# VatsalSy/gerris-fft-particles

Hardware: AMD Instinct MI355X
Metric: Mcell-steps/s (projection+advection), 3D 256^3 uniform (higher is better)
Workload: dtype f64; 1 GPU; 3-D periodic Taylor-Green, 256^3 per GPU, default projection/advection parameters (SURVEY 8d config C); relax_mode=exact, parallelism=1 box, rccl_world_size=0

## Files before the change

### gerris-fft-particles_amd/csrc/gfship_internal.hpp

```cpp
#pragma once

#include <hip/hip_runtime.h>
#include <cstdio>
#include <cstdarg>
#include <cstring>
#include <vector>
#include <deque>
#include <string>
#include <type_traits>
#include "gfship.h"
#include "switches.hpp"
#include "cell_update.hpp"

namespace gfship {

struct Layout {
  int n = 0;
  int px = 0;
  int xo = 1;
  int rows = 0;
  int dim = 3;
  long sy = 0;
  long sz = 0;
  size_t total = 0;
// ... 76 lines not shown
  double * h_pinned = nullptr;
  gfship_exchange_fn exchange = nullptr; void * exchange_ctx = nullptr;
  gfship_reduce_fn reduce = nullptr;     void * reduce_ctx = nullptr;
  bool has_external = false;
  void * comm = nullptr;
  int overlap = 0;
  int lat_rank = -1, lat_n = 0, lat_b[3] = { 1, 1, 1 };
  gfship_gather_fn gather = nullptr; void * gather_ctx = nullptr;
  double * lat_res = nullptr, * lat_xch = nullptr;
  unsigned * lat_bar = nullptr;
  size_t lat_res_doubles = 0, lat_xch_doubles = 0;
  double * gfv_send[6] = {}, * gfv_recv[6] = {};
  double src[3] = { 0., 0., 0. };
  unsigned long long n_lattice_cycles = 0, n_fused_mpi = 0;
  unsigned long long kc[GFSHIP_KC_COUNT] = {};
  bool lattice_attr_set = false;
  void * mpi_plan[GFSHIP_MAXLEVEL + 1] = {};
  gfship_field dp_cache = -1;
  int skew_resident = -1;
  int patch_resident = 0;
  bool no_fused_godunov = false;
  bool no_fused_loop = false;
  bool force_hyperplane = false;
  bool unit_weights = false;
  bool weighted = false;
  unsigned long weights_stamp = 0;
  gfship_field wf[6] = {-1, -1, -1, -1, -1, -1};
  gfship::SkewPlan skew[GFSHIP_MAXLEVEL + 1];
  double diff_w[GFSHIP_MAXLEVEL + 1] = {};
  double * cfl_partial = nullptr;
  size_t cfl_nblocks = 0, cfl_used = 0;
  bool cfl_dirty = false;
  bool coarse_attr_set = false;
  gfship_field res_cache = -1;
  bool diff_ready = false;
  int diff_kind = 1;
  int patch_call = -1;
};

namespace gfship {

void set_error (const char * fmt, ...);
int  hip_fail (hipError_t e, const char * what, const char * file, int line);

inline int before_write (gfship_domain * dom)
{
  return dom->before_write ? dom->before_write (dom->before_write_ctx) : GFSHIP_OK;
}

#define GFSHIP_HIP(call) do { hipError_t e_ = (call); \
    if (e_ != hipSuccess) return gfship::hip_fail (e_, #call, __FILE__, __LINE__); } while (0)

inline hipError_t stream_wait_spin (hipStream_t st)
{
  hipError_t e;
  while ((e = hipStreamQuery (st)) == hipErrorNotReady)
    ;
  return e;
}

template <class F> inline void with_bools (F && f) { f (); }
template <class F, class... B> inline void with_bools (F && f, bool b0, B... rest)
{
  if (b0) with_bools ([&] (auto... r) { f (std::true_type {}, r...); }, rest...);
  else    with_bools ([&] (auto... r) { f (std::false_type {}, r...); }, rest...);
}

template <class F, class... B> inline void with_kind (F && f, int kind, B... bools)
{
  auto k = [&] (auto K) { with_bools ([&] (auto... r) { f (K, r...); }, bools...); };
  if (kind == 3)      k (std::integral_constant<int, 3> {});
  else if (kind == 2) k (std::integral_constant<int, 2> {});
  else if (kind)      k (std::integral_constant<int, 1> {});
  else                k (std::integral_constant<int, 0> {});
}

#define GFSHIP_CHECK(cond, code, ...) do { if (!(cond)) { \
    gfship::set_error (__VA_ARGS__); return (code); } } while (0)

Field * get_field (gfship_domain * dom, gfship_field f);
int coarse_flush (gfship_domain * dom, Field * F, int level, bool leaf_write = false);
inline long ncells (const Layout & L) {
  return L.dim == 3 ? (long) L.n*L.n*L.n : (long) L.n*L.n;
}

int launch_bc (gfship_domain * dom, Field * v, Field * v1, int level, int homogeneous);
bool all_sides_periodic (const gfship_domain * dom);

__device__ __forceinline__ void periodic_images (const Layout & L, double * __restrict__ a, int i, int j, int k,
						  double v)
{
  const int n = L.n;
  if (i == 1) a[L.idx (n + 1, j, k)] = v;
  if (i == n) a[L.idx (0, j, k)] = v;
  if (j == 1) a[L.idx (i, n + 1, k)] = v;
  if (j == n) a[L.idx (i, 0, k)] = v;
  if (k == 1) a[L.idx (i, j, n + 1)] = v;
  if (k == n) a[L.idx (i, j, 0)] = v;
}
int call_exchange (gfship_domain * dom, double * ptr, int level, int kind);
int bc_mpi_begin (gfship_domain * dom, Field * v1, int level);
int bc_mpi_end (gfship_domain * dom, Field * v, Field * v1, int level, int homogeneous);
int call_reduce (gfship_domain * dom, double * vals, int n, int op);
int call_reduce_norm (gfship_domain * dom, double * sums, int nsum, double * mx);
int comm_exchange (gfship_domain * dom, double * a, int level, int kind);
int comm_exchange_raw (gfship_domain * dom, double * const send[6], double * const recv[6], size_t count);
int comm_migrate (gfship_domain * dom, int rs, const int nsend[6], const double * const send[6],
		  int nrecv[6], std::vector<double> recv[6]);
int comm_allgather (gfship_domain * dom, const double * send, double * recv, size_t count);
int multi_buffers (gfship_domain * dom);
int launch_bc_multi (gfship_domain * dom, Field * const * v, int nf, int level, int homogeneous);
int call_gather (gfship_domain * dom, const double * send, double * recv, size_t count);
int comm_exchange_begin (gfship_domain * dom, double * a, int level);
int comm_exchange_end (gfship_domain * dom, double * a, int level);
int comm_reduce (gfship_domain * dom, double * sums, int nsum, double * maxs, int nmax,
		 double * mins, int nmin);
void comm_free (gfship_domain * dom);
int launch_relax_exact (gfship_domain * dom, unsigned dimension, int level, double omega,
			double * u, const double * rhs, const double * dia,
			const RelaxOp * op = nullptr);
int launch_relax_mpi_first (gfship_domain * dom, unsigned dimension, int level, double omega,
			    double * u, const double * rhs, const double * dia, const RelaxOp * op,
			    int (* after_shell) (void *), void * ctx);
void mpi_order_free (gfship_domain * dom);
int launch_relax_loop_small (gfship_domain * dom, unsigned dimension, int level, double omega,
			     Field * dp, Field * ubc, const double * rhs, const double * dia,
			     unsigned nrelax, bool * done, const RelaxOp * op = nullptr);
int coarse_cycle_top (gfship_domain * dom, int minlevel);
int lattice_cycle_top (gfship_domain * dom, int minlevel, Field * dia);
int lattice_check_error (gfship_domain * dom);
int launch_lattice_cycle (gfship_domain * dom, unsigned dimension, double omega, int lmin, int ltop,
			  const unsigned * nrelax, Field * dp, Field * ubc, Field * res);
int launch_coarse_cycle (gfship_domain * dom, unsigned dimension, double omega, int lmin, int ltop,
			 const unsigned * nrelax, Field * dp, Field * ubc, Field * res, Field * dia);
int launch_relax_redblack (gfship_domain * dom, unsigned dimension, int level, double omega,
			   double * u, const double * rhs, const double * dia);
int launch_residual (gfship_domain * dom, int level, const double * u, const double * rhs,
		     const double * dia, double * res);
int launch_residual_weighted (gfship_domain * dom, int level, const double * u, const double * rhs,
			      const double * dia, double * res);
int launch_poisson_weights (gfship_domain * dom, double * const alpha[3]);
int launch_diffusion_weights (gfship_domain * dom, double * const D[3], double cdt);
int alloc_weights (gfship_domain * dom);
RelaxOp weighted_op (gfship_domain * dom, int level);
int launch_restrict (gfship_domain * dom, unsigned dimension, int level_coarse, double * v_coarse,
		     const double * v_fine);
int launch_prolongate (gfship_domain * dom, int level_coarse, const double * v_coarse,
		       double * v_fine);
int launch_correct (gfship_domain * dom, int level, double * u, const double * dp);
int launch_fill (gfship_domain * dom, int level, double * a, double value);
int launch_residual_norm (gfship_domain * dom, int level, const double * u, const double * rhs,
			  const double * dia, double * res, double scale, double weight,
			  double * out , bool dia_zero = false);
int launch_norm_async (gfship_domain * dom, int level, const double * a, double scale, double weight);
int launch_norm (gfship_domain * dom, int level, const double * a, double scale, double weight,
		 double out[5] );

int launch_face_interp_un (gfship_domain * dom, double * const u[3], double * const un[3]);
int launch_divergence (gfship_domain * dom, double * const un[3], double * div, double dt);
int launch_correct_un (gfship_domain * dom, const double * p, double * const un[3], double dt);
int launch_centered_gradient (gfship_domain * dom, const double * p, double * const g[3]);
int launch_correct_centered (gfship_domain * dom, double * const u[3], double * const g[3], double dt);
int launch_correct_centered_coarse (gfship_domain * dom, double * const u[3], double * const g[3],
				    double dt, double * const uc[3]);
int launch_coarse_init_from (gfship_domain * dom, Field * const * v, int nf, int top);
int launch_coarse_init_levels (gfship_domain * dom, Field * const * v, int nf, int top, int bottom);
// ... 84 lines not shown
```

### gerris-fft-particles_amd/csrc/poisson_kernels.hip

```cpp
#include "gfship_internal.hpp"
#include "cell_loop.hpp"
#include "relax_skew.hpp"
#include <algorithm>
#include <cstdlib>

namespace gfship {

template <int DIM, int OP>
__device__ __forceinline__ double relax_value (const double * __restrict__ u, long c, long sy, long sz,
					       double rhs, double dia, unsigned dimension,
					       double omega, double w, double h2, const W6 * wf = nullptr)
{
  return cell_update<DIM, OP> (kind_weights<OP> (w, ArrayW { wf, c }), ArrayU { u, c, sy, sz }, rhs, dia, u + c,
			       dimension, omega, h2);
}

__device__ __forceinline__ double relax_value_six (const double * __restrict__ u, long c, long sy, long sz,
						    double rhs)
{
  return cell_update_six (ArrayU { u, c, sy, sz }, rhs);
}

template <int DIM, int OP>
__global__ void __launch_bounds__(256)
// ... 1400 lines not shown
    for (int q = 0; q < 4; q++) {
      r0 += sh[0][q]; r1 += sh[1][q]; r2 += sh[2][q]; r3 = fmax (r3, sh[3][q]); r4 += sh[4][q];
    }
    out[0] = r0; out[1] = r1; out[2] = r2; out[3] = r3; out[4] = r4;
  }
}

static bool power_of_two (double x)
{
  int e;
  return x > 0. && frexp (x, &e) == 0.5;
}
#define NORM_PARTIAL_LAUNCH() do {					\
    if (power_of_two (scale))						\
      hipLaunchKernelGGL (norm_partial_kernel<true>, dim3 (nblocks), dim3 (block), 0, dom->stream, \
			  L, a, scale, weight, partial);		\
    else								\
      hipLaunchKernelGGL (norm_partial_kernel<false>, dim3 (nblocks), dim3 (block), 0, dom->stream, \
			  L, a, scale, weight, partial);		\
  } while (0)

int launch_norm_async (gfship_domain * dom, int level, const double * a, double scale, double weight)
{
  const Layout & L = dom->lay[level];
  long nrows = L.dim == 3 ? (long) L.n*L.n : L.n;
  int block = L.n >= 256 ? 256 : L.n >= 128 ? 128 : 64;
  int nblocks = (int) (nrows > 1024 ? 1024 : nrows);
  double * partial = dom->d_scratch;
  double * result = dom->h_pinned + 8;
  NORM_PARTIAL_LAUNCH ();
  hipLaunchKernelGGL (norm_final_kernel, dim3 (1), dim3 (256), 0, dom->stream,
		      partial, nblocks, result);
  GFSHIP_HIP (hipGetLastError ());
  return GFSHIP_OK;
}

int launch_norm (gfship_domain * dom, int level, const double * a, double scale, double weight,
		 double out[5])
{
  const Layout & L = dom->lay[level];
  long nrows = L.dim == 3 ? (long) L.n*L.n : L.n;
  int block = L.n >= 256 ? 256 : L.n >= 128 ? 128 : 64;
  int nblocks = (int) (nrows > 1024 ? 1024 : nrows);
  double * partial = dom->d_scratch;
  double * result = dom->h_pinned;
  NORM_PARTIAL_LAUNCH ();
  hipLaunchKernelGGL (norm_final_kernel, dim3 (1), dim3 (256), 0, dom->stream,
		      partial, nblocks, result);
  GFSHIP_HIP (hipGetLastError ());
  GFSHIP_HIP (stream_wait_spin (dom->stream));
  memcpy (out, dom->h_pinned, 5*sizeof (double));
  return GFSHIP_OK;
}

template <int DIM>
__global__ void __launch_bounds__(256)
residual_norm_kernel (Layout L, const double * __restrict__ u, const double * __restrict__ rhs,
		      const double * __restrict__ dia, double * __restrict__ res, double inv,
		      double weight, double * __restrict__ partial)
{
  const int n = L.n;
  const long nrows = DIM == 3 ? (long) n*n : n;
  double s0 = 0., s1 = 0., s2 = 0., s3 = 0., s4 = 0.;
  for (long r = blockIdx.x; r < nrows; r += gridDim.x) {
    const int j = (int) (r % n) + 1, k = DIM == 3 ? (int) (r / n) + 1 : 0;
    const long row = L.idx (1, j, k);
    for (int i = threadIdx.x; i < n; i += blockDim.x) {
      const long c = row + i;
      const FaceSums f = face_sums<DIM> (UnitW {}, ArrayU { u, c, L.sy, L.sz }, dia ? dia[c] : 0.);
      const double raw = residual_close (f.a, f.b, rhs[c], u[c]);
      res[c] = raw;
      double val = raw*inv;
      s0 += weight*val;
      val = fabs (val);
      s3 = fmax (s3, val);
      s1 += weight*val;
      s2 += weight*val*val;
      s4 += raw;
    }
  }
  block_norm_sums (s0, s1, s2, s3, s4, partial, blockIdx.x);
}

template <bool NORM>
__global__ void __launch_bounds__(256)
residual_norm2_kernel (Layout L, const double * __restrict__ u, const double * __restrict__ rhs,
		       const double * __restrict__ dia, double * __restrict__ res, double inv,
		       double weight, double * __restrict__ partial)
{
  typedef double d2 __attribute__((ext_vector_type(2)));
  const int n = L.n, half = n >> 1;
  const long nitems = (long) n*n*half;
  double s0 = 0., s1 = 0., s2 = 0., s3 = 0., s4 = 0.;
  for (long it = (long) blockIdx.x*blockDim.x + threadIdx.x; it < nitems; it += (long) gridDim.x*blockDim.x) {
    const int pr = (int) (it % half);
    const long r = it / half;
    const int j = (int) (r % n) + 1, k = (int) (r / n) + 1;
    const long c = L.idx (1 + 2*pr, j, k);
    const d2 uc = *(const d2 *) (u + c);
    const double ul = u[c - 1], ur = u[c + 2];
    const d2 ut = *(const d2 *) (u + c + L.sy), ub = *(const d2 *) (u + c - L.sy);
    const d2 uf = *(const d2 *) (u + c + L.sz), uk = *(const d2 *) (u + c - L.sz);
    const d2 rh = *(const d2 *) (rhs + c);
    d2 di = { 0., 0. };
    if (dia) di = *(const d2 *) (dia + c);
    d2 out;
    {
      double a = di.x, b = 0.;
      a += 1.; b += 1.*uc.y;
      a += 1.; b += 1.*ul;
      a += 1.; b += 1.*ut.x;
      a += 1.; b += 1.*ub.x;
      a += 1.; b += 1.*uf.x;
      a += 1.; b += 1.*uk.x;
      out.x = rh.x - (b - uc.x*a);
    }
    {
      double a = di.y, b = 0.;
      a += 1.; b += 1.*ur;
      a += 1.; b += 1.*uc.x;
      a += 1.; b += 1.*ut.y;
      a += 1.; b += 1.*ub.y;
      a += 1.; b += 1.*uf.y;
      a += 1.; b += 1.*uk.y;
      out.y = rh.y - (b - uc.y*a);
    }
    *(d2 *) (res + c) = out;
    if (NORM)
#pragma unroll
    for (int e = 0; e < 2; e++) {
      const double raw = e ? out.y : out.x;
      double val = raw*inv;
      s0 += weight*val;
      val = fabs (val);
      s3 = fmax (s3, val);
      s1 += weight*val;
      s2 += weight*val*val;
      s4 += raw;
    }
  }
  if (!NORM) return;
  __shared__ double sh[5][4];
  s0 = wave_sum (s0); s1 = wave_sum (s1); s2 = wave_sum (s2); s3 = wave_max (s3); s4 = wave_sum (s4);
  int w = threadIdx.x >> 6, lane = threadIdx.x & 63;
  if (lane == 0) { sh[0][w] = s0; sh[1][w] = s1; sh[2][w] = s2; sh[3][w] = s3; sh[4][w] = s4; }
  __syncthreads ();
  if (threadIdx.x == 0) {
    int nw = blockDim.x >> 6;
    double r0 = 0., r1 = 0., r2 = 0., r3 = 0., r4 = 0.;
    for (int q = 0; q < nw; q++) {
      r0 += sh[0][q]; r1 += sh[1][q]; r2 += sh[2][q]; r3 = fmax (r3, sh[3][q]); r4 += sh[4][q];
    }
    double * p = partial + 5*(size_t) blockIdx.x;
    p[0] = r0; p[1] = r1; p[2] = r2; p[3] = r3; p[4] = r4;
  }
}

int launch_residual_norm (gfship_domain * dom, int level, const double * u, const double * rhs,
			  const double * dia, double * res, double scale, double weight,
			  double * out, bool dia_zero)
{
  const Layout & L = dom->lay[level];
  if (!power_of_two (scale)) {
    int r = launch_residual (dom, level, u, rhs, dia, res);
    if (r) return r;
    return out ? launch_norm (dom, level, res, scale, weight, out) :
      launch_norm_async (dom, level, res, scale, weight);
  }
  long nrows = L.dim == 3 ? (long) L.n*L.n : L.n;
  int block = L.n >= 256 ? 256 : L.n >= 128 ? 128 : 64;
  int rn_blocks = dom->sw.rn_blocks;
  if (rn_blocks < 64 || rn_blocks > 8192) rn_blocks = 4096;
  int nblocks = (int) (nrows > rn_blocks ? rn_blocks : nrows);
  double * partial = dom->d_scratch;
  double * result = out ? dom->h_pinned : dom->h_pinned + 8;
  const bool rn_pairs = dom->sw.residual_pairs;
  if (dom->dim == 3 && L.n >= 64) dom->kc[rn_pairs ? GFSHIP_KC_RESIDUAL_PAIRS : GFSHIP_KC_RESIDUAL_SCALAR]++;
  if (dom->dim == 3 && L.n >= 64 && rn_pairs) {
    const long nitems = (long) L.n*L.n*(L.n/2);
    long nb = (nitems + 255)/256;
    nblocks = (int) (nb > rn_blocks ? rn_blocks : nb);
    hipLaunchKernelGGL (residual_norm2_kernel<true>, dim3 (nblocks), dim3 (256), 0, dom->stream, L, u,
			rhs, dia_zero ? nullptr : dia, res, 1./scale, weight, partial);
  }
  else
    with_bools ([&] (auto D3) {
      hipLaunchKernelGGL (residual_norm_kernel<decltype (D3)::value ? 3 : 2>, dim3 (nblocks), dim3 (block), 0,
			  dom->stream, L, u, rhs, dia_zero ? nullptr : dia, res, 1./scale, weight, partial);
    }, dom->dim == 3);
  hipLaunchKernelGGL (norm_final_kernel, dim3 (1), dim3 (256), 0, dom->stream,
		      partial, nblocks, result);
  GFSHIP_HIP (hipGetLastError ());
  dom->kc[GFSHIP_KC_RN_BLOCKS_LIMIT] = rn_blocks;
  if ((unsigned long long) nblocks > dom->kc[GFSHIP_KC_RN_BLOCKS_MAX])
    dom->kc[GFSHIP_KC_RN_BLOCKS_MAX] = nblocks;
  if (out) {
    GFSHIP_HIP (stream_wait_spin (dom->stream));
    memcpy (out, dom->h_pinned, 5*sizeof (double));
  }
  return GFSHIP_OK;
}

struct MpiOrderPlan {
  int * cells = nullptr;
  std::vector<int> first;
  int shell_steps = 0;
};

template <int DIM, int OP>
__global__ void __launch_bounds__(256)
relax_listed_kernel (const int * __restrict__ cells, int count, long sy, long sz,
		     unsigned dimension, double omega, double w, double h2,
		     double * __restrict__ u, const double * __restrict__ rhs,
		     const double * __restrict__ dia)
{
  const int q = blockIdx.x*blockDim.x + threadIdx.x;
  if (q >= count) return;
  const long c = cells[q];
  u[c] = relax_value<DIM, OP> (u, c, sy, sz, rhs[c], dia[c], dimension, omega, w, h2);
}

static inline unsigned long long morton_key (int dim, int level, int I, int J, int K)
{
  unsigned long long m = 0;
  for (int b = level - 1; b >= 0; b--) {
    unsigned n = ((I >> b) & 1) | (((J >> b) & 1) << 1) | (dim == 3 ? ((K >> b) & 1) << 2 : 0);
    m = (m << (dim == 3 ? 3 : 2)) | n;
  }
  return m;
}

void mpi_order_free (gfship_domain * dom)
{
  for (int l = 0; l <= GFSHIP_MAXLEVEL; l++)
    if (dom->mpi_plan[l]) {
      MpiOrderPlan * P = (MpiOrderPlan *) dom->mpi_plan[l];
// ... 121 lines not shown
```

### gerris-fft-particles_amd/csrc/timestep_kernels.hip

```cpp
#include "gfship_internal.hpp"
#include "cell_loop.hpp"
#include <cfloat>

namespace gfship {

#define EXT_PROLOGUE(L)							\
  int i = blockIdx.x*blockDim.x + threadIdx.x;				\
  int j = blockIdx.y;							\
  int k = (L).dim == 3 ? blockIdx.z : 0;				\
  if (i > (L).n) return;						\
  long c = (L).idx (i, j, k)

static inline void ext_grid (const Layout & L, dim3 * grid, dim3 * block)
{
  int b = L.n >= 256 ? 256 : L.n >= 128 ? 128 : 64;
  *block = dim3 (b);
  *grid = dim3 ((L.n + 1 + b - 1)/b, L.n + 1, L.dim == 3 ? L.n + 1 : 1);
}

struct Ptr3  { double * p[3]; };
struct CPtr3 { const double * p[3]; };
struct Ptr6  { double * p[6]; };
struct CPtr6 { const double * p[6]; };
struct Visc3 { double d[3]; double g[3]; };
// ... 107 lines not shown
	const long c = L.idx (2*i - 1, 2*j - dy, 2*k - dz);
	const d2 a = *(const d2 *) (u.p[cc] + c), b = *(const d2 *) (g.p[cc] + c);
	d2 r;
	r.x = a.x - b.x*dt; r.y = a.y - b.y*dt;
	*(d2 *) (u.p[cc] + c) = r;
	x[dz][dy][0] = r.x; x[dz][dy][1] = r.y;
      }
    double val = 0., sa = 0.;
#pragma unroll
    for (int id = 0; id < 8; id++) {
      val += x[(id >> 2) & 1][(id >> 1) & 1][id & 1]*1.;
      sa += 1.;
    }
    uc.p[cc][Lc.idx (i, j, k)] = val/sa;
  }
}

template <int DIM, bool FUSE_U>
__global__ void __launch_bounds__(256)
project_correct_kernel (Layout L, const double * __restrict__ p, Ptr3 un, Ptr3 g, Ptr3 u,
			double dt, double * __restrict__ partial_max)
{
  const int i1 = blockIdx.x*blockDim.x + threadIdx.x + 1;
  const int j = blockIdx.y;
  const int k = DIM == 3 ? blockIdx.z : 0;
  const int n = L.n;
  const double rn = (double) n;
  const long off[3] = { 1, L.sy, L.sz };
  double mx = 0.;
  auto body = [&] (int i) {
    const long c = L.idx (i, j, k);
    const bool interior = i >= 1 && j >= 1 && (DIM == 2 || k >= 1);
#pragma unroll
    for (int cc = 0; cc < DIM; cc++) {
      const bool valid = face_valid<DIM> (n, cc, i, j, k);
      if (valid || interior) {
	double dpp = (1.*p[c + off[cc]] - 1.*p[c])*rn;
	dpp /= 1.;
	if (valid) {
	  double w = un.p[cc][c];
	  w -= dpp*dt;
	  un.p[cc][c] = w;
	  mx = fmax (mx, fabs (w));
	}
	if (interior) {
	  double dpm = (1.*p[c] - 1.*p[c - off[cc]])*rn;
	  dpm /= 1.;
	  double v = 0.;
	  v += dpm*1.;
	  v += dpp*1.;
	  double gg = v/2.;
	  g.p[cc][c] = gg;
	  if (FUSE_U) {
	    double w = u.p[cc][c];
	    w -= gg*dt;
	    u.p[cc][c] = w;
	    mx = fmax (mx, fabs (1.*w));
	  }
	}
      }
    }
  };
  if (i1 <= n) {
    body (i1);
    if (i1 == 1)
      body (0);
  }
  if (partial_max) {
    __shared__ double sh[4];
    mx = wave_max (mx);
    if ((threadIdx.x & 63) == 0) sh[threadIdx.x >> 6] = mx;
    __syncthreads ();
    if (threadIdx.x == 0) {
      double r = sh[0];
      for (int q = 1; q < (int) (blockDim.x >> 6); q++) r = fmax (r, sh[q]);
      if (r > 0.)
	atomicMax ((unsigned long long *) partial_max +
		   ((blockIdx.x + gridDim.x*(blockIdx.y + (size_t) gridDim.y*blockIdx.z)) & 1023),
		   (unsigned long long) __double_as_longlong (r));
    }
  }
}

__global__ void __launch_bounds__(128)
face_interp_div2_kernel (Layout L, CPtr3 u, double * __restrict__ div, double dt)
{
  typedef double d2 __attribute__((ext_vector_type(2)));
  const int i1 = 2*(blockIdx.x*blockDim.x + threadIdx.x) + 1;
  const int j = blockIdx.y + 1, k = blockIdx.z + 1;
  if (i1 > L.n) return;
  const double h = 1./L.n;
  const long c = L.idx (i1, j, k);
  const long off[3] = { 1, L.sy, L.sz };
  d2 D = { 0., 0. };
#pragma unroll
  for (int cc = 0; cc < 3; cc++) {
    const d2 U = *(const d2 *) (u.p[cc] + c);
    d2 Un, Um;
    if (cc == 0) { Un.x = U.y; Un.y = u.p[0][c + 2]; Um.x = u.p[0][c - 1]; Um.y = U.x; }
    else { Un = *(const d2 *) (u.p[cc] + c + off[cc]); Um = *(const d2 *) (u.p[cc] + c - off[cc]); }
    {
      const double unp = face_interp (U.x, Un.x), unm = face_interp (Um.x, U.x);
      D.x += 1.*unp*1.;
      D.x += -1.*unm*1.;
    }
    {
      const double unp = face_interp (U.y, Un.y), unm = face_interp (Um.y, U.y);
      D.y += 1.*unp*1.;
      D.y += -1.*unm*1.;
    }
  }
  d2 out;
  { const double v = D.x*h; out.x = v/dt; }
  { const double v = D.y*h; out.y = v/dt; }
  *(d2 *) (div + c) = out;
}

__device__ __forceinline__ void periodic_images_pair (const Layout & L, double * __restrict__ a, long c,
						       int i1, int j, int k, double vx, double vy)
{
  typedef double d2 __attribute__((ext_vector_type(2)));
  const int n = L.n;
  const d2 V = { vx, vy };
  if (i1 == 1) a[c + n] = vx;
  if (i1 + 1 == n) a[c + 1 - n] = vy;
  if (j == 1) *(d2 *) (a + c + n*L.sy) = V;
  if (j == n) *(d2 *) (a + c - n*L.sy) = V;
  if (k == 1) *(d2 *) (a + c + n*L.sz) = V;
  if (k == n) *(d2 *) (a + c - n*L.sz) = V;
}

template <bool PER>
__global__ void __launch_bounds__(128)
project_correct2_kernel (Layout L, const double * __restrict__ p, Ptr3 un, Ptr3 g, double dt)
{
  typedef double d2 __attribute__((ext_vector_type(2)));
  const int i1 = 2*(blockIdx.x*blockDim.x + threadIdx.x) + 1;
  const int j = blockIdx.y, k = blockIdx.z;
  const int n = L.n;
  const double rn = (double) n;
  const long off[3] = { 1, L.sy, L.sz };
  auto body = [&] (int i) {
    const long c = L.idx (i, j, k);
    const bool interior = i >= 1 && j >= 1 && k >= 1;
#pragma unroll
    for (int cc = 0; cc < 3; cc++) {
      const bool valid = face_valid<3> (n, cc, i, j, k);
      if (valid || interior) {
	double dpp = (1.*p[c + off[cc]] - 1.*p[c])*rn;
	dpp /= 1.;
	if (valid) {
	  double w = un.p[cc][c];
	  w -= dpp*dt;
	  un.p[cc][c] = w;
	}
	if (interior) {
	  double dpm = (1.*p[c] - 1.*p[c - off[cc]])*rn;
	  dpm /= 1.;
	  double v = 0.;
	  v += dpm*1.;
	  v += dpp*1.;
	  g.p[cc][c] = v/2.;
	}
      }
    }
  };
  if (i1 > n) return;
  if (j >= 1 && k >= 1) {
    const long c = L.idx (i1, j, k);
    const d2 P = *(const d2 *) (p + c);
    const double pl = p[c - 1], pr = p[c + 2];
    const d2 Pn[3] = { { P.y, pr }, *(const d2 *) (p + c + L.sy), *(const d2 *) (p + c + L.sz) };
    const d2 Pm[3] = { { pl, P.x }, *(const d2 *) (p + c - L.sy), *(const d2 *) (p + c - L.sz) };
#pragma unroll
    for (int cc = 0; cc < 3; cc++) {
      d2 W = *(const d2 *) (un.p[cc] + c), G;
#pragma unroll
      for (int e = 0; e < 2; e++) {
	const double pc = e ? P.y : P.x, pn = e ? Pn[cc].y : Pn[cc].x, pm = e ? Pm[cc].y : Pm[cc].x;
	double dpp = (1.*pn - 1.*pc)*rn;
	dpp /= 1.;
	double w = e ? W.y : W.x;
	w -= dpp*dt;
	double dpm = (1.*pc - 1.*pm)*rn;
	dpm /= 1.;
	double v = 0.;
	v += dpm*1.;
	v += dpp*1.;
	if (e) { W.y = w; G.y = v/2.; } else { W.x = w; G.x = v/2.; }
      }
      *(d2 *) (un.p[cc] + c) = W;
      *(d2 *) (g.p[cc] + c) = G;
      if (PER) periodic_images_pair (L, g.p[cc], c, i1, j, k, G.x, G.y);
    }
  }
  else {
    body (i1);
    if (i1 + 1 <= n) body (i1 + 1);
  }
  if (i1 == 1)
    body (0);
}

template <bool PER>
__global__ void __launch_bounds__(128)
project_correct_lazy2_kernel (Layout L, const double * __restrict__ p, CPtr3 u, Ptr3 g, Ptr3 uo,
			      double dt, double * __restrict__ partial_max)
{
  typedef double d2 __attribute__((ext_vector_type(2)));
  const int i1 = 2*(blockIdx.x*blockDim.x + threadIdx.x) + 1;
  const int j = blockIdx.y, k = blockIdx.z;
  const int n = L.n;
  const double rn = (double) n;
  const long off[3] = { 1, L.sy, L.sz };
  double mx = 0.;
  auto body = [&] (int i) {
    const long c = L.idx (i, j, k);
    const bool interior = i >= 1 && j >= 1 && k >= 1;
#pragma unroll
    for (int cc = 0; cc < 3; cc++) {
      const bool valid = face_valid<3> (n, cc, i, j, k);
      if (valid || interior) {
	double dpp = (1.*p[c + off[cc]] - 1.*p[c])*rn;
	dpp /= 1.;
	const double uc = u.p[cc][c];
	if (valid) {
	  double w = face_interp (uc, u.p[cc][c + off[cc]]);
	  w -= dpp*dt;
	  mx = fmax (mx, fabs (w));
	}
	if (interior) {
	  double dpm = (1.*p[c] - 1.*p[c - off[cc]])*rn;
	  dpm /= 1.;
	  double v = 0.;
	  v += dpm*1.;
	  v += dpp*1.;
	  double gg = v/2.;
	  g.p[cc][c] = gg;
	  double w = uc;
	  w -= gg*dt;
	  uo.p[cc][c] = w;
	  mx = fmax (mx, fabs (1.*w));
	}
      }
    }
  };
  if (i1 <= n) {
    if (j >= 1 && k >= 1) {
      const long c = L.idx (i1, j, k);
      const d2 P = *(const d2 *) (p + c);
      const double pl = p[c - 1], pr = p[c + 2];
      const d2 Pn[3] = { { P.y, pr }, *(const d2 *) (p + c + L.sy), *(const d2 *) (p + c + L.sz) };
      const d2 Pm[3] = { { pl, P.x }, *(const d2 *) (p + c - L.sy), *(const d2 *) (p + c - L.sz) };
#pragma unroll
      for (int cc = 0; cc < 3; cc++) {
	const d2 U = *(const d2 *) (u.p[cc] + c);
	d2 Un;
	if (cc == 0) { Un.x = U.y; Un.y = u.p[0][c + 2]; }
	else Un = *(const d2 *) (u.p[cc] + c + off[cc]);
	d2 G, W;
#pragma unroll
	for (int e = 0; e < 2; e++) {
	  const double pc = e ? P.y : P.x, pn = e ? Pn[cc].y : Pn[cc].x, pm = e ? Pm[cc].y : Pm[cc].x;
	  const double uc = e ? U.y : U.x, un_ = e ? Un.y : Un.x;
	  double dpp = (1.*pn - 1.*pc)*rn;
	  dpp /= 1.;
	  double w = face_interp (uc, un_);
	  w -= dpp*dt;
	  mx = fmax (mx, fabs (w));
	  double dpm = (1.*pc - 1.*pm)*rn;
	  dpm /= 1.;
	  double v = 0.;
	  v += dpm*1.;
	  v += dpp*1.;
	  const double gg = v/2.;
	  double w2 = uc;
	  w2 -= gg*dt;
	  mx = fmax (mx, fabs (1.*w2));
	  if (e) { G.y = gg; W.y = w2; } else { G.x = gg; W.x = w2; }
	}
	*(d2 *) (g.p[cc] + c) = G;
	*(d2 *) (uo.p[cc] + c) = W;
	if (PER) {
	  periodic_images_pair (L, g.p[cc], c, i1, j, k, G.x, G.y);
	  periodic_images_pair (L, uo.p[cc], c, i1, j, k, W.x, W.y);
	}
      }
    }
    else {
      body (i1);
      if (i1 + 1 <= n) body (i1 + 1);
    }
    if (i1 == 1)
      body (0);
  }
  if (partial_max) {
    __shared__ double sh[4];
    mx = wave_max (mx);
    if ((threadIdx.x & 63) == 0) sh[threadIdx.x >> 6] = mx;
    __syncthreads ();
    if (threadIdx.x == 0) {
      double r = sh[0];
      for (int q = 1; q < (int) (blockDim.x >> 6); q++) r = fmax (r, sh[q]);
      if (r > 0.)
	atomicMax ((unsigned long long *) partial_max +
		   ((blockIdx.x + gridDim.x*(blockIdx.y + (size_t) gridDim.y*blockIdx.z)) & 1023),
		   (unsigned long long) __double_as_longlong (r));
    }
  }
}

struct W6t { const double * p[6]; };

template <int DIM>
__global__ void __launch_bounds__(256)
project_correct_weighted_kernel (Layout L, const double * __restrict__ p, Ptr3 un, Ptr3 g, Ptr3 u,
				 double dt, W6t wf)
{
  const int i1 = blockIdx.x*blockDim.x + threadIdx.x + 1;
  const int j = blockIdx.y;
  const int k = DIM == 3 ? blockIdx.z : 0;
  const int n = L.n;
  const double rn = (double) n;
  const long off[3] = { 1, L.sy, L.sz };
  auto body = [&] (int i) {
    const long c = L.idx (i, j, k);
    const int q[3] = { i, j, k };
    const bool interior = i >= 1 && j >= 1 && (DIM == 2 || k >= 1);
#pragma unroll
    for (int cc = 0; cc < DIM; cc++) {
      const bool valid = face_valid<DIM> (n, cc, i, j, k);
      if (valid || interior) {
	const double wp = q[cc] >= 1 ? wf.p[2*cc][c] : wf.p[2*cc + 1][c + off[cc]];
	double dpp = (wp*p[c + off[cc]] - wp*p[c])*rn;
	dpp /= 1.;
	if (valid && un.p[cc]) {
	  double w = un.p[cc][c];
	  w -= dpp*dt;
	  un.p[cc][c] = w;
	}
	if (interior) {
	  const double wm = q[cc] >= 2 ? wf.p[2*cc][c - off[cc]] : wf.p[2*cc + 1][c];
	  double dpm = (wm*p[c] - wm*p[c - off[cc]])*rn;
	  dpm /= 1.;
	  double v = 0.;
	  v += dpm*1.;
	  v += dpp*1.;
	  double gg = v/2.;
	  g.p[cc][c] = gg;
	  if (u.p[cc]) {
	    double w = u.p[cc][c];
	    w -= gg*dt;
	    u.p[cc][c] = w;
	  }
	}
      }
    }
  };
  if (i1 <= n) {
    body (i1);
    if (i1 == 1)
      body (0);
  }
}

template <int DIM>
__global__ void __launch_bounds__(256)
project_correct_lazy_kernel (Layout L, const double * __restrict__ p, CPtr3 u, Ptr3 g, Ptr3 uo,
			     double dt, double * __restrict__ partial_max)
{
  const int i1 = blockIdx.x*blockDim.x + threadIdx.x + 1;
  const int j = blockIdx.y;
  const int k = DIM == 3 ? blockIdx.z : 0;
  const int n = L.n;
  const double rn = (double) n;
  const long off[3] = { 1, L.sy, L.sz };
  double mx = 0.;
  auto body = [&] (int i) {
    const long c = L.idx (i, j, k);
    const bool interior = i >= 1 && j >= 1 && (DIM == 2 || k >= 1);
#pragma unroll
    for (int cc = 0; cc < DIM; cc++) {
      const bool valid = face_valid<DIM> (n, cc, i, j, k);
      if (valid || interior) {
	double dpp = (1.*p[c + off[cc]] - 1.*p[c])*rn;
	dpp /= 1.;
	const double uc = u.p[cc][c];
	if (valid) {
	  double w = face_interp (uc, u.p[cc][c + off[cc]]);
// ... 2262 lines not shown
  dim3 grid ((nface + block - 1)/block, 2*dom->dim);
  DISPATCH (dom, face_bc_kernel, grid, dim3 (block), L, bc, (const double *) v->lev[dom->depth],
	    m6 (fv), cmask);
  if (dom->has_external)
    for (int e = 0; e < 2*dom->dim; e++)
      if (dom->side[e ^ 1] == GFSHIP_SIDE_EXTERNAL && (cmask & (1 << (e/2)))) {
	int r = call_exchange (dom, fv[e], dom->depth, 1 + e);
	if (r) return r;
      }
  return GFSHIP_OK;
}

int launch_predict_un (gfship_domain * dom, int cc, const double * uc, double * const fv[6],
		       double * unc)
{
  const Layout & L = dom->lay[dom->depth];
  dim3 grid, block;
  ext_grid (L, &grid, &block);
  DISPATCH (dom, predict_un_kernel, grid, block, L, cc, uc, (const double *) fv[2*cc],
	    (const double *) fv[2*cc + 1], unc);
  return GFSHIP_OK;
}

int launch_flux_update (gfship_domain * dom, bool velocity, double * v, double * const un[3],
			double * const fv[6], const double * gm, const double * gc, double dt, double gsrc)
{
  const Layout & L = dom->lay[dom->depth];
  dim3 grid, block;
  cell_grid (L, &grid, &block);
  if (dom->dim == 3) {
    if (velocity)
      hipLaunchKernelGGL ((flux_update_kernel<3, true>), grid, block, 0, dom->stream,
			  L, v, c3 (un), c6 (fv), gm, gc, dt, gsrc);
    else
      hipLaunchKernelGGL ((flux_update_kernel<3, false>), grid, block, 0, dom->stream,
			  L, v, c3 (un), c6 (fv), gm, gc, dt, gsrc);
  }
  else {
    if (velocity)
      hipLaunchKernelGGL ((flux_update_kernel<2, true>), grid, block, 0, dom->stream,
			  L, v, c3 (un), c6 (fv), gm, gc, dt, gsrc);
    else
      hipLaunchKernelGGL ((flux_update_kernel<2, false>), grid, block, 0, dom->stream,
			  L, v, c3 (un), c6 (fv), gm, gc, dt, gsrc);
  }
  GFSHIP_HIP (hipGetLastError ());
  return GFSHIP_OK;
}

static inline void ext1_grid (const Layout & L, dim3 * grid, dim3 * block)
{
  int b = L.n >= 256 ? 256 : L.n >= 128 ? 128 : 64;
  *block = dim3 (b);
  *grid = dim3 ((L.n + b - 1)/b, L.n + 1, L.dim == 3 ? L.n + 1 : 1);
}

int launch_project_correct (gfship_domain * dom, const double * p, double * const un[3],
			    double * const g[3], double * const u[3] , double dt,
			    bool want_max, bool * ghosts_done)
{
  if (ghosts_done) *ghosts_done = false;
  const Layout & L = dom->lay[dom->depth];
  dim3 grid, block;
  ext1_grid (L, &grid, &block);
  double * pm = nullptr;
  if (want_max) {
    const size_t nb = 1024;
    if (!dom->cfl_partial) {
      GFSHIP_HIP (hipMalloc ((void **) &dom->cfl_partial, nb*sizeof (double)));
      GFSHIP_HIP (hipMemsetAsync (dom->cfl_partial, 0, nb*sizeof (double), dom->stream));
      dom->cfl_nblocks = nb;
    }
    dom->cfl_used = nb;
    if (dom->cfl_dirty)
      GFSHIP_HIP (hipMemsetAsync (dom->cfl_partial, 0, nb*sizeof (double), dom->stream));
    dom->cfl_dirty = true;
    pm = dom->cfl_partial;
  }
  Ptr3 none = { { nullptr, nullptr, nullptr } };
  const bool pairs = dom->sw.project_pairs;
  const bool pairs_apply = dom->dim == 3 && !u && !pm && L.n >= 64 && L.n % 2 == 0;
  if (pairs_apply) dom->kc[pairs ? GFSHIP_KC_PROJECT_PAIRS : GFSHIP_KC_PROJECT_SCALAR]++;
  if (pairs_apply && pairs) {
    const int b = 128, half = L.n/2;
    const bool per = ghosts_done && all_sides_periodic (dom);
    with_bools ([&] (auto PER) {
      hipLaunchKernelGGL (project_correct2_kernel<decltype (PER)::value>, dim3 ((half + b - 1)/b, L.n + 1, L.n + 1), dim3 (b), 0,
			  dom->stream, L, p, m3 (un), m3 (g), dt);
    }, per);
    GFSHIP_HIP (hipGetLastError ());
    if (per) *ghosts_done = true;
    return GFSHIP_OK;
  }
  with_bools ([&] (auto D3, auto U) {
    hipLaunchKernelGGL ((project_correct_kernel<decltype (D3)::value ? 3 : 2, decltype (U)::value>), grid, block, 0, dom->stream,
			L, p, m3 (un), m3 (g), u ? m3 (u) : none, dt, pm);
  }, dom->dim == 3, u != nullptr);
  GFSHIP_HIP (hipGetLastError ());
  return GFSHIP_OK;
}

int launch_project_correct_weighted (gfship_domain * dom, const double * p, double * const un[3] ,
				     double * const g[3], double * const u[3] , double dt)
{
  const int Lv = dom->depth;
  const Layout & L = dom->lay[Lv];
  dim3 grid, block;
  ext1_grid (L, &grid, &block);
  W6t wf;
  for (int d = 0; d < 6; d++)
    wf.p[d] = d < 2*dom->dim ? dom->fields[dom->wf[d]].lev[Lv] : nullptr;
  Ptr3 none = { { nullptr, nullptr, nullptr } };
  if (dom->dim == 3)
    hipLaunchKernelGGL ((project_correct_weighted_kernel<3>), grid, block, 0, dom->stream, L, p,
			un ? m3 (un) : none, m3 (g), u ? m3 (u) : none, dt, wf);
  else
    hipLaunchKernelGGL ((project_correct_weighted_kernel<2>), grid, block, 0, dom->stream, L, p,
			un ? m3 (un) : none, m3 (g), u ? m3 (u) : none, dt, wf);
  GFSHIP_HIP (hipGetLastError ());
  return GFSHIP_OK;
}

int launch_cfl_from_max (gfship_domain * dom, double * cfl2)
{
  const Layout & L = dom->lay[dom->depth];
  double * result = dom->h_pinned;
  hipLaunchKernelGGL (cfl_from_max_kernel, dim3 (1), dim3 (256), 0, dom->stream, dom->cfl_partial,
		      (int) dom->cfl_used, 1./L.n, result);
  dom->cfl_dirty = false;
  GFSHIP_HIP (hipGetLastError ());
  GFSHIP_HIP (stream_wait_spin (dom->stream));
  *cfl2 = dom->h_pinned[0];
  return call_reduce (dom, cfl2, 1, 2);
}

int launch_face_interp_div (gfship_domain * dom, double * const u[3], double * const un[3],
			    double * div, double dt)
{
  const Layout & L = dom->lay[dom->depth];
  dim3 grid, block;
  ext1_grid (L, &grid, &block);
  Ptr3 none = { { nullptr, nullptr, nullptr } };
  const bool pairs = dom->sw.project_pairs;
  const bool pairs_apply = !un && dom->dim == 3 && L.n >= 64 && L.n % 2 == 0;
  if (pairs_apply) dom->kc[pairs ? GFSHIP_KC_PROJECT_PAIRS : GFSHIP_KC_PROJECT_SCALAR]++;
  if (pairs_apply && pairs) {
    const int b = 128, half = L.n/2;
    hipLaunchKernelGGL (face_interp_div2_kernel, dim3 ((half + b - 1)/b, L.n, L.n), dim3 (b), 0, dom->stream, L, c3 (u), div, dt);
  }
  else
    with_bools ([&] (auto D3, auto UN) {
      hipLaunchKernelGGL ((face_interp_div_kernel<decltype (D3)::value ? 3 : 2, decltype (UN)::value>), grid, block, 0, dom->stream,
			  L, c3 (u), un ? m3 (un) : none, div, dt);
    }, dom->dim == 3, un != nullptr);
  GFSHIP_HIP (hipGetLastError ());
  return GFSHIP_OK;
}

int launch_project_correct_lazy (gfship_domain * dom, const double * p, double * const u[3],
				 double * const g[3], double * const uo[3], double dt, bool * ghosts_done)
{
  if (ghosts_done) *ghosts_done = false;
  const Layout & L = dom->lay[dom->depth];
  dim3 grid, block;
  ext1_grid (L, &grid, &block);
  const size_t nb = 1024;
  if (!dom->cfl_partial) {
    GFSHIP_HIP (hipMalloc ((void **) &dom->cfl_partial, nb*sizeof (double)));
    GFSHIP_HIP (hipMemsetAsync (dom->cfl_partial, 0, nb*sizeof (double), dom->stream));
    dom->cfl_nblocks = nb;
  }
  dom->cfl_used = nb;
  if (dom->cfl_dirty)
    GFSHIP_HIP (hipMemsetAsync (dom->cfl_partial, 0, nb*sizeof (double), dom->stream));
  dom->cfl_dirty = true;
  const bool pairs = dom->sw.project_pairs;
  const bool pairs_apply = dom->dim == 3 && L.n >= 64 && L.n % 2 == 0;
  if (pairs_apply) dom->kc[pairs ? GFSHIP_KC_PROJECT_PAIRS : GFSHIP_KC_PROJECT_SCALAR]++;
  if (pairs_apply && pairs) {
    const int b = 128, half = L.n/2;
    const bool per = ghosts_done && all_sides_periodic (dom);
    with_bools ([&] (auto PER) {
      hipLaunchKernelGGL (project_correct_lazy2_kernel<decltype (PER)::value>, dim3 ((half + b - 1)/b, L.n + 1, L.n + 1), dim3 (b), 0,
			  dom->stream, L, p, c3 (u), m3 (g), m3 (uo), dt, dom->cfl_partial);
    }, per);
    if (per) *ghosts_done = true;
  }
  else if (dom->dim == 3)
    hipLaunchKernelGGL ((project_correct_lazy_kernel<3>), grid, block, 0, dom->stream, L, p, c3 (u), m3 (g), m3 (uo), dt, dom->cfl_partial);
  else
    hipLaunchKernelGGL ((project_correct_lazy_kernel<2>), grid, block, 0, dom->stream, L, p, c3 (u), m3 (g), m3 (uo), dt, dom->cfl_partial);
  GFSHIP_HIP (hipGetLastError ());
  return GFSHIP_OK;
}

bool godunov_fused_supported (const gfship_domain * dom)
{
  if (dom->dim != 3 || dom->no_fused_godunov) return false;
  const int n = dom->lay[dom->depth].n;
  if (n % GX) return false;
  for (int d = 0; d < 6; d++)
    if (dom->side[d] != GFSHIP_SIDE_PERIODIC) return false;
  return true;
}

bool godunov_fused_mpi_supported (const gfship_domain * dom)
{
  if (dom->dim != 3 || dom->no_fused_godunov || !dom->sw.fused_mpi || !dom->comm) return false;
  const int n = dom->lay[dom->depth].n;
  if (n % GX) return false;
  bool ext = false;
  for (int d = 0; d < 6; d++) {
    if (dom->side[d] == GFSHIP_SIDE_EXTERNAL) ext = true;
    else if (dom->side[d] != GFSHIP_SIDE_PERIODIC) return false;
  }
  return ext;
}

static int ghost_fv (gfship_domain * dom, GhostFv * G)
{
  if (int r = multi_buffers (dom)) return r;
  for (int d = 0; d < 6; d++) {
    G->r[d] = nullptr; G->s[d] = nullptr;
    if (dom->side[d] != GFSHIP_SIDE_EXTERNAL) continue;
    G->s[d] = dom->gfv_send[d];
    G->r[d] = dom->gfv_recv[d];
  }
  return GFSHIP_OK;
}

int launch_predict_un_fused (gfship_domain * dom, double * const u[3], double dt, int gradient,
			     const double visc[3], double * const un[3], double * div, double div_dt,
			     bool * div_done)
{
  const Layout & L = dom->lay[dom->depth];
  Visc3 vs;
  for (int c = 0; c < 3; c++) { vs.d[c] = visc[c]; vs.g[c] = dom->src[c]; }
  const bool anyv = visc[0] != 0. || visc[1] != 0. || visc[2] != 0. ||
    dom->src[0] != 0. || dom->src[1] != 0. || dom->src[2] != 0.;
  if (div_done) *div_done = false;
  GhostFv G;
  for (int d = 0; d < 6; d++) { G.r[d] = nullptr; G.s[d] = nullptr; }
  const bool mpi = dom->has_external;
  if (mpi) {
    int r = ghost_fv (dom, &G);
    if (r) return r;
    const dim3 bgrid ((L.n*L.n + 255)/256, 6);
    CPtr3 none = { { nullptr, nullptr, nullptr } };
    with_bools ([&] (auto VL, auto VS) {
      hipLaunchKernelGGL ((boundary_face_values_kernel<true, decltype (VL)::value, decltype (VS)::value>), bgrid, dim3 (256), 0,
			  dom->stream, L, c3 (u), none, dt, vs, G);
    }, gradient != 0, anyv);
    GFSHIP_HIP (hipGetLastError ());
    if ((r = comm_exchange_raw (dom, dom->gfv_send, dom->gfv_recv, (size_t) L.n*L.n))) return r;
    dom->n_fused_mpi++;
  }
  const bool sweep_fits = dom->sw.advect_sweep && L.n % SWX == 0 && L.n % SWY == 0 && L.n % SWZ == 0;
  if (sweep_fits && (!mpi || dom->sw.mpi_sweep)) {
    const dim3 sgrid (L.n/SWX, L.n/SWY, L.n/SWZ);
    const bool dv = div != nullptr && div_dt != 0.;
    with_bools ([&] (auto VL, auto VS, auto DV, auto MPI) {
      hipLaunchKernelGGL ((predict_un_sweep_kernel<decltype (VL)::value, decltype (VS)::value, decltype (DV)::value, decltype (MPI)::value>),
			  sgrid, dim3 (SWN + SW_RING), 0, dom->stream, L, c3 (u), m3 (un), dt, vs, div, div_dt, G);
    }, gradient != 0, anyv, dv, mpi);
    GFSHIP_HIP (hipGetLastError ());
    dom->kc[mpi ? GFSHIP_KC_PREDICT_SWEEP_MPI : GFSHIP_KC_PREDICT_SWEEP]++;
// ... 165 lines not shown
```

Before: 2693 Mcell-steps/s.

## Remap block indices into per-XCD contiguous slabs for stencil kernels

Adds an XCD-aware block remapping so that blocks dispatched round-robin to the eight XCDs each work on a contiguous j/k slab. The goal is to keep stencil neighbour rows in the same XCD's L2 instead of spreading them across XCDs. It is applied by default to the residual-norm kernel and the face-interp divergence kernel. The projection kernels now use a flattened 1-D grid, but their slab mapping is compiled off. The index arithmetic adds some per-block integer work and depends on the dispatch order being round-robin.

```diff
diff --git a/gerris-fft-particles_amd/csrc/gfship_internal.hpp b/gerris-fft-particles_amd/csrc/gfship_internal.hpp
--- a/gerris-fft-particles_amd/csrc/gfship_internal.hpp
+++ b/gerris-fft-particles_amd/csrc/gfship_internal.hpp
@@ -182,6 +182,36 @@
 int coarse_flush (gfship_domain * dom, Field * F, int level, bool leaf_write = false);
 inline long ncells (const Layout & L) {
   return L.dim == 3 ? (long) L.n*L.n*L.n : (long) L.n*L.n;
+}
+
+struct SlabRow { int j, k; };
+constexpr int XCD_CLASSES = 8;
+
+__host__ __device__ inline SlabRow xcd_slab_row (int block, int nblocks, int nrows_j, int nrows_k, int rows_per_block)
+{
+  const int nbj = (nrows_j + rows_per_block - 1)/rows_per_block;
+  const int wslab = ((nrows_j + XCD_CLASSES - 1)/XCD_CLASSES + rows_per_block - 1)/rows_per_block;
+  const int q = nblocks/XCD_CLASSES, r = nblocks % XCD_CLASSES, c = block % XCD_CLASSES;
+  int place = (c < r ? c*(q + 1) : r*(q + 1) + (c - r)*q) + block/XCD_CLASSES;
+  const int full = nblocks/nbj, rest = nblocks % nbj;
+  (void) nrows_k;
+  for (int s = 0; s < XCD_CLASSES; s++) {
+    int w = nbj - s*wslab;
+    w = w < 0 ? 0 : w > wslab ? wslab : w;
+    int e = rest - s*wslab;
+    e = e < 0 ? 0 : e > w ? w : e;
+    const int size = w*full + e;
+    if (place < size)
+      return SlabRow { (s*wslab + place % w)*rows_per_block, place/w };
+    place -= size;
+  }
+  return SlabRow { 0, 0 };
+}
+
+__host__ __device__ inline int xcd_slab_block (int block, int nblocks, int nrows_j, int nrows_k, int rows_per_block)
+{
+  const SlabRow s = xcd_slab_row (block, nblocks, nrows_j, nrows_k, rows_per_block);
+  return s.j/rows_per_block + (nrows_j + rows_per_block - 1)/rows_per_block*s.k;
 }
 
 int launch_bc (gfship_domain * dom, Field * v, Field * v1, int level, int homogeneous);
diff --git a/gerris-fft-particles_amd/csrc/poisson_kernels.hip b/gerris-fft-particles_amd/csrc/poisson_kernels.hip
--- a/gerris-fft-particles_amd/csrc/poisson_kernels.hip
+++ b/gerris-fft-particles_amd/csrc/poisson_kernels.hip
@@ -1506,6 +1506,9 @@
   block_norm_sums (s0, s1, s2, s3, s4, partial, blockIdx.x);
 }
 
+#ifndef XS_RESIDUAL
+#define XS_RESIDUAL 1
+#endif
 template <bool NORM>
 __global__ void __launch_bounds__(256)
 residual_norm2_kernel (Layout L, const double * __restrict__ u, const double * __restrict__ rhs,
@@ -1516,7 +1519,9 @@
   const int n = L.n, half = n >> 1;
   const long nitems = (long) n*n*half;
   double s0 = 0., s1 = 0., s2 = 0., s3 = 0., s4 = 0.;
-  for (long it = (long) blockIdx.x*blockDim.x + threadIdx.x; it < nitems; it += (long) gridDim.x*blockDim.x) {
+  const int rpb = half < 256 ? 256/half : 1;
+  const int bid = XS_RESIDUAL ? xcd_slab_block (blockIdx.x, gridDim.x, (int) ((long) n*half*rpb/256), n, rpb) : blockIdx.x;
+  for (long it = (long) bid*blockDim.x + threadIdx.x; it < nitems; it += (long) gridDim.x*blockDim.x) {
     const int pr = (int) (it % half);
     const long r = it / half;
     const int j = (int) (r % n) + 1, k = (int) (r / n) + 1;
@@ -1575,7 +1580,7 @@
     for (int q = 0; q < nw; q++) {
       r0 += sh[0][q]; r1 += sh[1][q]; r2 += sh[2][q]; r3 = fmax (r3, sh[3][q]); r4 += sh[4][q];
     }
-    double * p = partial + 5*(size_t) blockIdx.x;
+    double * p = partial + 5*(size_t) bid;
     p[0] = r0; p[1] = r1; p[2] = r2; p[3] = r3; p[4] = r4;
   }
 }
diff --git a/gerris-fft-particles_amd/csrc/timestep_kernels.hip b/gerris-fft-particles_amd/csrc/timestep_kernels.hip
--- a/gerris-fft-particles_amd/csrc/timestep_kernels.hip
+++ b/gerris-fft-particles_amd/csrc/timestep_kernels.hip
@@ -213,12 +213,34 @@
   }
 }
 
+#ifndef XS_FACE_DIV
+#define XS_FACE_DIV 1
+#endif
+#ifndef XS_PROJECT
+#define XS_PROJECT 0
+#endif
+#ifndef XS_PROJECT_LAZY
+#define XS_PROJECT_LAZY 0
+#endif
+struct PairBlock { int bx, j, k, plain; };
+
+__device__ __forceinline__ PairBlock pair_block (bool slabs, int n, int rows, int b)
+{
+  const int gx = (n/2 + b - 1)/b;
+  SlabRow s = { (int) (blockIdx.x % (unsigned) (gx*rows)), (int) (blockIdx.x / (unsigned) (gx*rows)) };
+  if (slabs) s = xcd_slab_row (blockIdx.x, gridDim.x, gx*rows, rows, 1);
+  return PairBlock { s.j % gx, s.j / gx, s.k, s.j + gx*rows*s.k };
+}
+
+inline dim3 pair_grid (int n, int rows, int b) { return dim3 ((n/2 + b - 1)/b*rows*rows); }
+
 __global__ void __launch_bounds__(128)
 face_interp_div2_kernel (Layout L, CPtr3 u, double * __restrict__ div, double dt)
 {
   typedef double d2 __attribute__((ext_vector_type(2)));
-  const int i1 = 2*(blockIdx.x*blockDim.x + threadIdx.x) + 1;
-  const int j = blockIdx.y + 1, k = blockIdx.z + 1;
+  const PairBlock pb = pair_block (XS_FACE_DIV, L.n, L.n, blockDim.x);
+  const int i1 = 2*(pb.bx*blockDim.x + threadIdx.x) + 1;
+  const int j = pb.j + 1, k = pb.k + 1;
   if (i1 > L.n) return;
   const double h = 1./L.n;
   const long c = L.idx (i1, j, k);
@@ -266,9 +288,10 @@
 project_correct2_kernel (Layout L, const double * __restrict__ p, Ptr3 un, Ptr3 g, double dt)
 {
   typedef double d2 __attribute__((ext_vector_type(2)));
-  const int i1 = 2*(blockIdx.x*blockDim.x + threadIdx.x) + 1;
-  const int j = blockIdx.y, k = blockIdx.z;
   const int n = L.n;
+  const PairBlock pb = pair_block (XS_PROJECT, n, n + 1, blockDim.x);
+  const int i1 = 2*(pb.bx*blockDim.x + threadIdx.x) + 1;
+  const int j = pb.j, k = pb.k;
   const double rn = (double) n;
   const long off[3] = { 1, L.sy, L.sz };
   auto body = [&] (int i) {
@@ -339,9 +362,10 @@
 			      double dt, double * __restrict__ partial_max)
 {
   typedef double d2 __attribute__((ext_vector_type(2)));
-  const int i1 = 2*(blockIdx.x*blockDim.x + threadIdx.x) + 1;
-  const int j = blockIdx.y, k = blockIdx.z;
   const int n = L.n;
+  const PairBlock pb = pair_block (XS_PROJECT_LAZY, n, n + 1, blockDim.x);
+  const int i1 = 2*(pb.bx*blockDim.x + threadIdx.x) + 1;
+  const int j = pb.j, k = pb.k;
   const double rn = (double) n;
   const long off[3] = { 1, L.sy, L.sz };
   double mx = 0.;
@@ -434,8 +458,7 @@
       double r = sh[0];
       for (int q = 1; q < (int) (blockDim.x >> 6); q++) r = fmax (r, sh[q]);
       if (r > 0.)
-	atomicMax ((unsigned long long *) partial_max +
-		   ((blockIdx.x + gridDim.x*(blockIdx.y + (size_t) gridDim.y*blockIdx.z)) & 1023),
+	atomicMax ((unsigned long long *) partial_max + (pb.plain & 1023),
 		   (unsigned long long) __double_as_longlong (r));
     }
   }
@@ -2864,10 +2887,10 @@
   const bool pairs_apply = dom->dim == 3 && !u && !pm && L.n >= 64 && L.n % 2 == 0;
   if (pairs_apply) dom->kc[pairs ? GFSHIP_KC_PROJECT_PAIRS : GFSHIP_KC_PROJECT_SCALAR]++;
   if (pairs_apply && pairs) {
-    const int b = 128, half = L.n/2;
+    const int b = 128;
     const bool per = ghosts_done && all_sides_periodic (dom);
     with_bools ([&] (auto PER) {
-      hipLaunchKernelGGL (project_correct2_kernel<decltype (PER)::value>, dim3 ((half + b - 1)/b, L.n + 1, L.n + 1), dim3 (b), 0,
+      hipLaunchKernelGGL (project_correct2_kernel<decltype (PER)::value>, pair_grid (L.n, L.n + 1, b), dim3 (b), 0,
 			  dom->stream, L, p, m3 (un), m3 (g), dt);
     }, per);
     GFSHIP_HIP (hipGetLastError ());
@@ -2927,8 +2950,8 @@
   const bool pairs_apply = !un && dom->dim == 3 && L.n >= 64 && L.n % 2 == 0;
   if (pairs_apply) dom->kc[pairs ? GFSHIP_KC_PROJECT_PAIRS : GFSHIP_KC_PROJECT_SCALAR]++;
   if (pairs_apply && pairs) {
-    const int b = 128, half = L.n/2;
-    hipLaunchKernelGGL (face_interp_div2_kernel, dim3 ((half + b - 1)/b, L.n, L.n), dim3 (b), 0, dom->stream, L, c3 (u), div, dt);
+    const int b = 128;
+    hipLaunchKernelGGL (face_interp_div2_kernel, pair_grid (L.n, L.n, b), dim3 (b), 0, dom->stream, L, c3 (u), div, dt);
   }
   else
     with_bools ([&] (auto D3, auto UN) {
@@ -2960,10 +2983,10 @@
   const bool pairs_apply = dom->dim == 3 && L.n >= 64 && L.n % 2 == 0;
   if (pairs_apply) dom->kc[pairs ? GFSHIP_KC_PROJECT_PAIRS : GFSHIP_KC_PROJECT_SCALAR]++;
   if (pairs_apply && pairs) {
-    const int b = 128, half = L.n/2;
+    const int b = 128;
     const bool per = ghosts_done && all_sides_periodic (dom);
     with_bools ([&] (auto PER) {
-      hipLaunchKernelGGL (project_correct_lazy2_kernel<decltype (PER)::value>, dim3 ((half + b - 1)/b, L.n + 1, L.n + 1), dim3 (b), 0,
+      hipLaunchKernelGGL (project_correct_lazy2_kernel<decltype (PER)::value>, pair_grid (L.n, L.n + 1, b), dim3 (b), 0,
 			  dom->stream, L, p, c3 (u), m3 (g), m3 (uo), dt, dom->cfl_partial);
     }, per);
     if (per) *ghosts_done = true;
```

Result: no change. 2682 Mcell-steps/s (-0.4%).
